# dkogan/libdogleg

Measured on AMD Instinct MI355X. Metric: trust-region steps/sec (fp64) at fixed (Nmeas,Nstate,nnz), higher is better.
Workload: dtype f64

## Files before the change

libdogleg_amd/capi.py:

```python
import ctypes as C
import os
import numpy as np

from .ctypes_defs import (Parameters2, CholmodSparse, Trace, TraceBuffer, BatchResult, BatchLoss, BatchBounds, BatchFit, JacobianReport, JacobianEntry,
                          CB_SPARSE, CB_DENSE, CB_PRODUCTS, dptr, iptr)

HERE = os.path.dirname(os.path.abspath(__file__))
LIB_PATH = os.environ.get("DLG_TEST_LIB") or os.path.join(HERE, "libdogleg_amd.so")

DLG_OK = 0
DLG_DENSE, DLG_SPARSE, DLG_DENSE_PRODUCTS = 0, 1, 2
FLAG_PACKED, FLAG_UPPER = 1, 2
KIND_CAUCHY, KIND_GN, KIND_INTERP = 0, 1, 2
VEC_P, VEC_X, VEC_JTX, VEC_CAUCHY, VEC_GN, VEC_STEP, VEC_J, VEC_X_OWN, VEC_J_OWN = range(9)

ALLREDUCE_FN = C.CFUNCTYPE(C.c_int, C.c_void_p, C.c_size_t, C.c_void_p)

BACKEND_SYMBOLS = [
    "dlg_last_error", "dlg_device_count", "dlg_backend_create", "dlg_backend_destroy",
    "dlg_backend_set_stream", "dlg_backend_get_stream", "dlg_backend_set_shard",
    "dlg_sparse_set_pattern", "dlg_sparse_stats", "dlg_sparse_schedule", "dlg_sparse_leaf_rows_stats", "dlg_point_set_p", "dlg_point_upload",
    "dlg_point_upload_products", "dlg_point_bind_device", "dlg_point_eval", "dlg_cauchy",
    "dlg_factorize", "dlg_solve_gn", "dlg_gauss_newton", "dlg_cauchy_gauss_newton", "dlg_make_step",
    "dlg_expected_improvement", "dlg_step", "dlg_take_step", "dlg_solve_with_factor",
# ... 832 lines not shown

    def init_rccl(self, rank, nranks, unique_id):
        buf = C.create_string_buffer(unique_id, 128)
        _ck(self.L.dlg_backend_init_rccl(self.h, rank, nranks, C.cast(buf, C.c_void_p)), "init_rccl")

    def set_noop_comm(self, on=True):
        _ck(self.L.dlg_backend_set_noop_comm(self.h, 1 if on else 0), "set_noop_comm")

    def comm_size(self):
        n = C.c_int()
        _ck(self.L.dlg_backend_comm_size(self.h, C.byref(n)), "comm_size")
        return n.value

    def set_pattern(self, Jp, Ji):
        Jp = np.ascontiguousarray(Jp, dtype=np.int32)
        Ji = np.ascontiguousarray(Ji, dtype=np.int32)
        _ck(self.L.dlg_sparse_set_pattern(self.h, iptr(Jp), iptr(Ji)), "set_pattern")

    def stats(self):
        a, b = C.c_long(), C.c_long()
        c, d = C.c_int(), C.c_int()
        e = C.c_double()
        _ck(self.L.dlg_sparse_stats(self.h, C.byref(a), C.byref(b), C.byref(c), C.byref(d), C.byref(e)),
            "stats")
        return dict(nnz_JtJ_lower=a.value, nnz_L=b.value, n_supernodes=c.value, n_levels=d.value,
                    factor_flops=e.value)

    def schedule(self):
        a, b, c = C.c_int(), C.c_int(), C.c_int()
        _ck(self.L.dlg_sparse_schedule(self.h, C.byref(a), C.byref(b), C.byref(c)), "schedule")
        return dict(n_levels=a.value, persist_level0=b.value, persist_items=c.value)

    def leaf_rows_stats(self):
        v = (C.c_long * 4)()
        _ck(self.L.dlg_sparse_leaf_rows_stats(self.h, v, 4), "leaf_rows_stats")
        return dict(lean_launches=v[0], materialized=v[1], raw=bool(v[2]), lean_levels=v[3])

    def set_p(self, slot, p):
        p = np.ascontiguousarray(p, dtype=np.float64)
        _ck(self.L.dlg_point_set_p(self.h, slot, dptr(p)), "set_p")

    def upload(self, slot, x, J):
        x = np.ascontiguousarray(x, dtype=np.float64)
        J = np.ascontiguousarray(J, dtype=np.float64)
        self._keep = [x, J]
        _ck(self.L.dlg_point_upload(self.h, slot, dptr(x), dptr(J)), "upload")

    def upload_products(self, slot, norm2x, Jtx, JtJ):
        Jtx = np.ascontiguousarray(Jtx, dtype=np.float64)
        JtJ = np.ascontiguousarray(JtJ, dtype=np.float64)
        self._keep = [Jtx, JtJ]
        _ck(self.L.dlg_point_upload_products(self.h, slot, norm2x, dptr(Jtx), dptr(JtJ)), "upload")

    def bind_device(self, slot, x_ptr, J_ptr):
        _ck(self.L.dlg_point_bind_device(self.h, slot, C.c_void_p(x_ptr), C.c_void_p(J_ptr)), "bind")

    def eval(self, slot):
        a, b = C.c_double(), C.c_double()
        _ck(self.L.dlg_point_eval(self.h, slot, C.byref(a), C.byref(b)), "eval")
        return a.value, b.value

    def cauchy(self, slot):
        a = C.c_double()
        _ck(self.L.dlg_cauchy(self.h, slot, C.byref(a)), "cauchy")
        return a.value

    def factorize(self, slot, lam=0.0):
        ok = C.c_int()
        _ck(self.L.dlg_factorize(self.h, slot, lam, C.byref(ok)), "factorize")
# ... 199 lines not shown
```

libdogleg_amd/csrc/backend.hip:

```cpp
#include "dlg_internal.h"

static thread_local char g_err[1024] = "";
#include <chrono>
#include <atomic>
#include <mutex>
namespace {
constexpr int DLG_TURN_DEV = 64;
std::mutex g_turn_mu;
std::atomic<int> g_turn_live[DLG_TURN_DEV];
hipEvent_t g_turn_ev[DLG_TURN_DEV];
dlg_backend* g_turn_owner[DLG_TURN_DEV];
}
DlgRegionTurn::DlgRegionTurn(dlg_backend* b_) : b(b_), on(false)
{
  const int d = b->device & (DLG_TURN_DEV - 1);
  if(g_turn_live[d].load(std::memory_order_relaxed) <= 1 || !b->ev_region) return;
  on = true;
  g_turn_mu.lock();
  if(g_turn_owner[d] && g_turn_owner[d] != b && g_turn_ev[d]) (void)hipEventSynchronize(g_turn_ev[d]);
}
DlgRegionTurn::~DlgRegionTurn()
{
  if(!on) return;
  const int d = b->device & (DLG_TURN_DEV - 1);
// ... 175 lines not shown

  auto fail = [&](int rc) { dlg_backend_destroy(b); return rc; };
#define TRY_HIP(call) do { hipError_t e_ = (call); if(e_ != hipSuccess) { \
    dlg_set_error("%s:%d: %s -> %s", __FILE__, __LINE__, #call, hipGetErrorString(e_)); \
    return fail(DLG_ERR_HIP); } } while(0)

  TRY_HIP(hipStreamCreateWithFlags(&b->stream, hipStreamNonBlocking));
  b->own_stream = true;
  TRY_HIP(hipStreamCreateWithFlags(&b->copy_stream, hipStreamNonBlocking));
  TRY_HIP(hipEventCreateWithFlags(&b->ev_step, hipEventDisableTiming));
  TRY_HIP(hipEventCreateWithFlags(&b->ev_copy, hipEventDisableTiming));
  TRY_HIP(hipStreamCreateWithFlags(&b->aux_stream, hipStreamNonBlocking));
  TRY_HIP(hipEventCreateWithFlags(&b->ev_fork, hipEventDisableTiming));
  TRY_HIP(hipEventCreateWithFlags(&b->ev_join, hipEventDisableTiming));
  TRY_HIP(hipEventCreateWithFlags(&b->ev_region, hipEventDisableTiming));
  turn_register(b); b->turn_registered = true;
  TRY_HIP(hipMalloc(&b->d_join, sizeof(int)*2));
  TRY_HIP(hipMemsetAsync(b->d_join, 0, sizeof(int)*2, b->stream));
  b->overlap = getenv("DOGLEG_AMD_NO_OVERLAP") == nullptr;
  b->fuse_eval = getenv("DOGLEG_AMD_NO_FUSED_EVAL") == nullptr;
  TRY_HIP(hipMalloc(&b->d_scal, sizeof(double)*dlg_backend::NSCAL));
  TRY_HIP(hipMemsetAsync(b->d_scal, 0, sizeof(double)*dlg_backend::NSCAL, b->stream));
  TRY_HIP(hipHostMalloc(&b->h_scal, sizeof(double)*dlg_backend::NSCAL));
  TRY_HIP(hipHostMalloc(&b->h_part, sizeof(double)*dlg_backend::HPART_CAP));
  b->host_finals = getenv("DOGLEG_AMD_DEVICE_FINALS") == nullptr;
  {
    dlg_backend::Knobs& k = b->knobs;
    k.potrf_steps = getenv("DOGLEG_AMD_POTRF_STEPS") != nullptr;
    k.trsv_steps = getenv("DOGLEG_AMD_TRSV_STEPS") != nullptr;
    k.no_abandon = getenv("DOGLEG_AMD_NO_ABANDON") != nullptr;
    k.ei_jpass = getenv("DOGLEG_AMD_EI_JPASS") != nullptr;
    k.no_between = getenv("DOGLEG_AMD_NO_BETWEEN") != nullptr;
    k.no_k8_predict = getenv("DOGLEG_AMD_NO_K8_PREDICT") != nullptr;
    if(const char* e = getenv("DOGLEG_AMD_DEBUG_EI_FLIP")) b->ei_flip = atoi(e);
    if(getenv("DOGLEG_AMD_DEBUG_HANDOFF_TIMEOUT")) { b->handoff_skew = 1; b->handoff_spins = 256; }
    (void)hipDeviceGetAttribute(&b->ncu, hipDeviceAttributeMultiprocessorCount, device);
    if(b->ncu <= 0) b->ncu = 256;
  }
  TRY_HIP(hipHostMalloc(&b->h_vec, sizeof(double)*(size_t)Nstate));
  TRY_HIP(hipMalloc(&b->d_work, sizeof(double)*(size_t)Nstate));
  const size_t N = (size_t)Nstate, M = (size_t)Nmeas;
  for(int s = 0; s < 2; s++)
  {
    DlgSlot& S = b->slot[s];
    TRY_HIP(hipMalloc(&S.p,      sizeof(double)*N));
    TRY_HIP(hipMalloc(&S.Jt_x,   sizeof(double)*(N + 8)));
    TRY_HIP(hipMalloc(&S.cauchy, sizeof(double)*N));
    TRY_HIP(hipMalloc(&S.gn,     sizeof(double)*(N + 8)));
    TRY_HIP(hipMalloc(&S.step,   sizeof(double)*N));
    TRY_HIP(hipMemsetAsync(S.p, 0, sizeof(double)*N, b->stream));
    TRY_HIP(hipMemsetAsync(S.step, 0, sizeof(double)*N, b->stream));
    if(solve_type != DLG_DENSE_PRODUCTS && M > 0) TRY_HIP(hipMalloc(&S.x, sizeof(double)*M));
    TRY_HIP(hipMalloc(&S.J, sizeof(double)*dlg_j_doubles(b)));
  }
#undef TRY_HIP
  int rc = (solve_type == DLG_SPARSE) ? sparse_create(b) : dense_create(b);
  if(rc != DLG_OK) return fail(rc);
  if(hipStreamSynchronize(b->stream) != hipSuccess)
  { dlg_set_error("stream sync failed during create"); return fail(DLG_ERR_HIP); }
  *out = b;
  return DLG_OK;
}

extern "C" void dlg_backend_destroy(dlg_backend_t* b)
{
  if(!b) return;
// ... 372 lines not shown
```

libdogleg_amd/csrc/dlg_internal.h:

```cpp
#pragma once
#include <hip/hip_runtime.h>
#include <hip/hip_ext.h>
#include <cstdio>
#include <cstdlib>
#include <cstring>
#include <cstdarg>
#include <cmath>
#include <vector>
#include <string>
#include "../../include/dlg_backend.h"

void dlg_set_error(const char* fmt, ...);

#define DLG_HIP(call)                                                              \
  do {                                                                             \
    hipError_t e__ = (call);                                                       \
    if(e__ != hipSuccess) {                                                        \
      dlg_set_error("%s:%d: %s -> %s", __FILE__, __LINE__, #call,                  \
                    hipGetErrorString(e__));                                       \
      return DLG_ERR_HIP;                                                          \
    }                                                                              \
  } while(0)

#define DLG_CHECK(call)                                                            \
// ... 43 lines not shown
  bool presolve = false;
  bool pre_rejected = false;
  bool factor_ahead = false;
  bool pre_split = false;
  bool prof_cont = false;
  int  pre_slot = -1, pre_held = -1; double pre_lambda = 0.0, pre_hint = 0.0; bool pre_hint_valid = false, pre_hint_input = false;
  DlgSlot slot[2];

  double* d_scal = nullptr;
  double* h_scal = nullptr;
  int* fork_gate = nullptr; int fork_gate_epoch = 0;
  bool defer_tail = false, tail_pending = false;
  int tail_nb = 0;
  double tail_inner = 0.0, tail_value = 0.0;
  double* h_tail = nullptr; int h_tail_cap = 0;
  unsigned long sync_mark = 0, tail_mark = 0;
  bool factor_doomed = false;
  static constexpr int IDENT_SLOT = 3, GB_SLOT = 13;
  static constexpr double IDENT_RATIO_MAX = 212.0;
  static constexpr double IDENT_ERR_MAX = 1e-12;
  bool ident_predict = false;
  bool ei_from_system = false; double pivot_ratio = NAN;
  int ei_flip = 0, ei_count = 0;
  bool tail_ident = false, tail_no_fold = false; double tail_nJs = 0.0;
  bool p_side_pending = false;
  dlg_between_fn between_fn = nullptr; void* between_cookie = nullptr; bool between_armed = false, between_ran = false, between_redone = false;
  int early_slot = -1; const double* early_x = nullptr; const double* early_J = nullptr;
  static constexpr int NSCAL = 16;
  int handoff_spins = 0, handoff_skew = 0;
  struct Knobs
  {
    bool potrf_steps = false, trsv_steps = false, no_abandon = false, ei_jpass = false, no_between = false, no_k8_predict = false;
    int touch_wg = 512;
  } knobs;
  int ncu = 256;

  double* d_part = nullptr;
  size_t  part_cap = 0;
  double* d_gnpart = nullptr;
  struct PendingFinal { size_t off; int nb, nsum, nmax, dst, stride; };
  static constexpr size_t HPART_CAP = 16384;
  double* h_part = nullptr;
  size_t  h_part_used = 0;
  std::vector<PendingFinal> pending;
  bool    host_finals = true;

  double* h_vec = nullptr;

  double* G = nullptr;
  double* Linv = nullptr;
  int* potrf_flag = nullptr; int potrf_epoch = 0; int* trsv_flag = nullptr; double* trsv_y = nullptr; double* trsv_x = nullptr; int trsv_epoch = 0;
  double* slabs = nullptr;
  size_t  slabs_bytes = 0;
  int*    d_info = nullptr;
  int*    h_info = nullptr;
  bool    defer_factor_sync = false;
  double* d_work = nullptr;
  DevScratch solve_scr, lev_scr;
  struct CovPlan* cov = nullptr; int cov_last = -1;
  struct SelInv* selinv = nullptr;

  SparseSym* sym = nullptr;

  int row0 = 0, row1 = 0;
  int mloc = 0;
  int part_rank = 0, part_nranks = 1;
// ... 287 lines not shown
```

libdogleg_amd/csrc/sparse_factor.hip:

```cpp
#include "sparse_internal.h"
#include "panel_factor.h"
#include "factor_tail.h"

namespace {
#ifdef DLG_FL_PROFILE
constexpr int FL_PROF_WG = 4096;
__device__ long long g_fl_prof[32*FL_PROF_WG*8];
__device__ long long g_fl_add[FL_PROF_WG*4];
#define FL_ADD_STAMP(k) do { if(HANDOFF && threadIdx.x == 0 && blockIdx.x < FL_PROF_WG) g_fl_add[blockIdx.x*4 + (k)] = wall_clock64(); } while(0)
#define FL_STAMP(k) do { if(threadIdx.x == 0 && blockIdx.x < FL_PROF_WG) g_fl_prof[((prof_lvl & 31)*FL_PROF_WG + blockIdx.x)*8 + (k)] = wall_clock64(); } while(0)
#else
#define FL_STAMP(k)
#define FL_ADD_STAMP(k)
#endif

template <int NT, bool UT_LDS, bool HANDOFF = false>
__device__ __forceinline__ void mf_add_children(double* P, double* Wt, int ntri, int nch, int ch0,
                                                MfChild rc, const MfChild* __restrict__ mf_rec,
                                                const double* uscr, const uint16_t* __restrict__ mf_dst, int tid,
                                                int* pr_flag = nullptr, int pr_epoch = 0, DlgHandoff ho = DlgHandoff{nullptr, 0, 0}, int z0 = 0)
{
  constexpr int MF_SLOTS = (NT >= 512) ? 20 : 16;
  const int lane = tid & 63;
  for(int e = z0 + tid; e < ntri; e += NT) Wt[e] = 0.0;
// ... 1196 lines not shown
                         Y->upart, (const int*)Y->d_info);
    if(H.part_nranks > 1 && l == H.cut_level) { DLG_LAUNCH_CHECK(); DLG_CHECK(sparse_partition_reduce(b)); }
  }
  if(!H.ms_sn.empty())
    hipLaunchKernelGGL(k_copy_top, dim3((unsigned)H.ms_sn.size()), dim3(TPB), 0, st, Y->ms_sn, Y->sn_c0,
                       Y->sn_rowptr, Y->sn_lx, Y->sn_top, Y->Lx, Y->top_scr, (const int*)Y->d_info);
  DLG_LAUNCH_CHECK();
  return DLG_OK;
}

int sparse_leaf_rows_materialize(dlg_backend* b)
{
  SparseSym* Y = b->sym;
  if(!Y || !Y->Lx || !Y->leaf_rows.raw(Y->Lx)) return DLG_OK;
  const SymHost& H = Y->H;
  const int slot = Y->leaf_rows.slot(Y->Lx);
  for(int l = 0; l < H.nlevels; l++)
  {
    const int n = H.fw_lvl_ptr[l+1] - H.fw_lvl_ptr[l];
    if(!Y->leaf_lean[l] || n == 0) continue;
    hipLaunchKernelGGL(HIP_KERNEL_NAME(k_leaf_rows_materialize<256>), dim3(n), dim3(256), Y->fac.lds[l], b->stream,
                       Y->fw_item + H.fw_lvl_ptr[l], Y->Lx, Y->leaf_rd + (size_t)slot*H.N, (const int*)Y->d_info);
  }
  DLG_LAUNCH_CHECK();
  Y->leaf_rows.materialize(Y->Lx);
  return DLG_OK;
}
extern "C" int dlg_sparse_leaf_rows_stats(dlg_backend_t* b, long* stats, int nstats)
{
  if(!b || !b->sym || !stats) { dlg_set_error("no symbolic analysis yet"); return DLG_ERR_STATE; }
  const SparseSym* Y = b->sym;
  long lean = 0;
  for(char c : Y->leaf_lean) lean += c;
  const long v[] = { Y->leaf_rows.lean_launches, Y->leaf_rows.materialized, Y->leaf_rows.raw(Y->Lx) ? 1L : 0L, lean };
  for(int i = 0; i < nstats && i < 4; i++) stats[i] = v[i];
  return DLG_OK;
}

extern "C" int dlg_sparse_region_probe(int N, int M, const int* colptr, const int* rowidx, int ncu, long* stats, int nstats)
{
  SymHost H;
  char err[512];
  if(sym_analyze(H, N, M, colptr, rowidx, 0, M, err, sizeof(err))) { dlg_set_error("symbolic analysis: %s", err); return DLG_ERR_ARG; }
  const RegionKnobs K = region_knobs_env(ncu);
  FacLevels L;
  if(fac_level_params(H, L, err, sizeof(err))) { dlg_set_error("%s", err); return DLG_ERR_ARG; }
  const RegionPlan R = region_plan(H, L, 1, H.nlevels - 1, K);
  long checked[2];
  if(region_check(H, R, checked, err, sizeof(err))) { dlg_set_error("%s", err); return DLG_ERR_STATE; }
  const long v[] = { (long)R.level0, (long)(H.fw_lvl_ptr[H.nlevels] - H.fw_lvl_ptr[std::min(R.level0, H.nlevels)]),
                     (long)R.nwg, (long)R.lds, checked[0], checked[1], (long)region_plan_hash(R), (long)fac_levels_hash(L) };
  for(int i = 0; i < nstats && i < 8; i++) stats[i] = v[i];
  return DLG_OK;
}
```

libdogleg_amd/csrc/sparse_internal.h:

```cpp
#pragma once
#include "dlg_internal.h"
#include "sparse_symbolic.h"
#include "sparse_region.h"
#include "leaf_rows_state.h"

namespace {
constexpr int JFL_SEG = 16;
constexpr int NV_CHUNK = 2048;

constexpr int TPB = 256;
constexpr int LDS_BUDGET = SYM_LDS_BUDGET;
constexpr int FAC_LDS_BUDGET = SYM_FAC_LDS_BUDGET;

__device__ __forceinline__ double wave_sum(double v)
{
#pragma unroll
  for(int o = 32; o > 0; o >>= 1) v += __shfl_down(v, o, 64);
  return v;
}

template <int NT, int U, class LoadF, class StoreF>
__device__ __forceinline__ void batched_copy(int total, int tid, LoadF ld, StoreF st)
{
  for(int base = 0; base < total; base += U*NT)
// ... 45 lines not shown
  int *jtx_fin_ptr = nullptr, *jtx_fin_blk = nullptr;
  int *jtx_fin_short = nullptr, *jtx_fin_long = nullptr; int n_fin_short = 0, n_fin_long = 0;
  AsmRho* asm_rho = nullptr; AsmPair* asm_pair = nullptr; AsmSlot* asm_slot = nullptr;
  AsmBatch* asm_batch = nullptr; AsmTask* asm_ctask = nullptr; AsmFin* asm_cfin = nullptr;
  bool asm_pent_ok = false;
  uint32_t* asm_pent = nullptr;
  AsmShape* asm_shape = nullptr; AsmKG* asm_kg = nullptr; AsmMTask* asm_mtask = nullptr; int* asm_tdest = nullptr;
  int *jf_ptr = nullptr, *jf_ent = nullptr, *jf_var0 = nullptr, *jf_w = nullptr, *jf_short = nullptr, *jf_long = nullptr;
  double* jf_lpart = nullptr; int* jf_lcnt = nullptr;
  const double* fin_pending_rhs = nullptr; const double* spec_aug_rhs = nullptr; bool info_clean = false;
  double* fin_pending_Lx = nullptr;
  bool spare_dirty = false, spare_zeroed = false; hipStream_t spare_stream = nullptr;
  double* jtp = nullptr;
  AsmFin2* asm_fin2 = nullptr; int64_t* asm_fin2_list = nullptr; AsmRun* asm_run = nullptr; int* asm_pdest = nullptr;
  int *rl_ptr = nullptr, *rl_pos = nullptr, *perm = nullptr, *col_sn = nullptr;
  int *fw_sn = nullptr, *fw_r0 = nullptr, *fw_r1 = nullptr, *ms_sn = nullptr; int64_t* sn_top = nullptr;
  int *sn_bd_ptr = nullptr, *sn_bd_col = nullptr;
  double* top_scr = nullptr;
  const double* aug_rhs = nullptr;
  int *Jp = nullptr, *Ji = nullptr;
  int *gat_rows = nullptr, *gat_src = nullptr;
  int *nv_chunk = nullptr; int n_nv_chunks = 0;
  double *Lx = nullptr, *scr = nullptr, *ywork = nullptr, *asm_part = nullptr, *jtx_part = nullptr;
  int *d_info = nullptr, *h_info = nullptr;
  bool info_armed = false;
  bool zero_fail_seen = false; int64_t* leaf_diag = nullptr; int* leaf_diag_col = nullptr; int n_leaf_diag = 0;
  double* intact_Lx = nullptr; const double* intact_J = nullptr; int intact_slot = -1; double intact_lambda = 0.0;
  const double* fac_J = nullptr; int fac_slot = -1;
  bool fac_pending = false;
  size_t nnz_loc = 0;
  uint32_t* ar_idx = nullptr; double* ar_buf = nullptr; size_t ar_n = 0;
  FacLevels fac;
  std::vector<int> slv_lds, bwd_lds, bwd_nt, bwd_bd, bwd_pmx;
  int64_t* red_off = nullptr; int* red_len = nullptr; int* red_kind = nullptr; int64_t* red_dst = nullptr;
  int n_red_seg = 0; size_t red_n = 0; double* red_buf = nullptr;
  double* colmask = nullptr; int* sn_owner = nullptr;
  int64_t* augpos = nullptr;
  int *xl_sn = nullptr;
  double* held_Lx = nullptr; const double* held_aug = nullptr; double held_lambda = 0.0;
  LeafRowsState leaf_rows; std::vector<char> leaf_lean; double* leaf_rd = nullptr;
  double cur_lambda = 0.0;
  double *ms_scr = nullptr, *ms_y = nullptr; int ms_lds_f = 0, ms_lds_b = 0;
  typedef ReachPlan LevPlan;
  LevPlan lev[2];
  int* lev_iperm = nullptr; std::vector<int> lev_jp, lev_ji; int lev_lds = 0;
  double* Lx_spec = nullptr; hipEvent_t ev_spec = nullptr, ev_spec_fork = nullptr;
  bool spec_inflight = false, spec_valid = false; int spec_slot = -1; const double* spec_J = nullptr;
  int64_t touch_off = 0, touch_n = 0;
  int bw_level0 = 1 << 30, bw_lds = 0, bw_n = 0;
  SolveItem* slv_item_pr = nullptr; int* bwd_flag = nullptr; int bwd_epoch = 0; double* bwd_xh = nullptr;
  PrRegion top, lo; double* pr_acc = nullptr;
  int64_t* clr_off = nullptr; int64_t* clr_len = nullptr; int n_clr = 0; bool clr_partial_ok = false; double* lz_ok[2] = {nullptr, nullptr};
  int64_t* aug_of_var = nullptr; char* jf_listed = nullptr;
  int aug_fused_epoch = 0; const double* spec_aug_fused = nullptr;
  int* fin_flag = nullptr; int fin_epoch = 0, fin_side_owed = 0; bool fin_side_sched_ok = false; hipStream_t fin_main = nullptr;
  int bwd_xb_cap = 12288;
  double* diag_mm = nullptr; int n_diag_mm = 0;
  std::vector<void*> allocs;
};

int sparse_assemble(dlg_backend* b, int s, double lambda);
int sparse_partition_reduce(dlg_backend* b);
int sparse_assemble_speculative(dlg_backend* b, int s);
int sparse_eval_assemble(dlg_backend* b, int s, int* done);
int sparse_assemble_finish(dlg_backend* b);
int sparse_zero_spare(dlg_backend* b, hipStream_t ordered_for);
// ... 5 lines not shown
```

libdogleg_amd/csrc/sparse_solve.hip:

```cpp
#include "sparse_internal.h"

namespace {
#ifdef DLG_FL_PROFILE
__device__ long long g_bw_prof[64*8];
__device__ long long g_bw_chain[256*8];
#define BW_STAMP(k) do { if(threadIdx.x == 0 && blockIdx.x == 0) g_bw_prof[(prof_lvl & 63)*8 + (k)] = clock64(); \
                         if(threadIdx.x == 0 && pr_flag && blockIdx.x < 256) g_bw_chain[blockIdx.x*8 + (k)] = wall_clock64(); } while(0)
#else
#define BW_STAMP(k)
#endif

__global__ void __launch_bounds__(TPB) k_solve_fwd_level(const int* __restrict__ lvl_sn,
                                                         const int* __restrict__ sn_c0,
                                                         const int* __restrict__ sn_rowptr,
                                                         const int64_t* __restrict__ sn_lx,
                                                         const int* __restrict__ sn_scr,
                                                         const int* __restrict__ rl_ptr,
                                                         const int* __restrict__ rl_pos,
                                                         const int* __restrict__ perm,
                                                         const double* __restrict__ Lx,
                                                         const double* __restrict__ rhs,
                                                         double* __restrict__ scr,
                                                         double* __restrict__ ywork)
{
// ... 31 lines not shown
      __syncthreads();
      if(lane == 0) red[wv] = sum;
      __syncthreads();
      if(tid == 0) y[j] = rhs[perm[k]] - ((red[0] + red[1]) + (red[2] + red[3]));
    }
    else if((j & 3) == wv)
    {
      double sum = 0.0;
      for(int e = e0 + lane; e < e1; e += 64) sum += scr[rl_pos[e]];
      sum = wave_sum(sum);
      if(lane == 0) y[j] = rhs[perm[k]] - sum;
    }
  }
  __syncthreads();
  double yi = (tid < w) ? y[tid] : 0.0;
  for(int j = 0; j < w; j++)
  {
    if(tid == j) y[j] = yi / lds[j + j*ldp];
    __syncthreads();
    if(tid > j && tid < w) yi -= lds[tid + j*ldp]*y[j];
  }
  __syncthreads();
  for(int j = tid; j < w; j += TPB) ywork[c0 + j] = y[j];
  const int r = nrows - w - 1;
  double* u = scr + sn_scr[s];
  for(int i = tid; i < r; i += TPB)
  {
    double sum = 0.0;
#pragma unroll 8
    for(int j = 0; j < w; j++) sum += L[w + i + (size_t)j*nrows]*y[j];
    u[i] = sum;
  }
}
template <int BWD_NT, bool BD_ONLY>
__global__ void __launch_bounds__(BWD_NT, BD_ONLY ? 4 : 1) k_solve_bwd_level(const SolveItem* __restrict__ items,
                                                            const int* __restrict__ sn_rows,
                                                            const int* __restrict__ perm,
                                                            const double* __restrict__ Lx,
                                                            double* __restrict__ ywork,
                                                            double* __restrict__ out, int use_aug,
                                                            const int* __restrict__ sn_bd_col, int top_lds, int xb_cap,
                                                            int* pr_flag, int pr_epoch, const int* __restrict__ info, DlgHandoff ho,
                                                            double* xh, int xh_n, double* __restrict__ mm, int rows_raw)
{
  extern __shared__ __attribute__((aligned(16))) double lds[];
  __shared__ int s_skip;
  double dmin = 1e300, dmax = 0.0;
  if(threadIdx.x == 0) s_skip = *info != 0x7fffffff;
  constexpr int NW = BWD_NT/64;
  typedef const __attribute__((address_space(1))) double* gcd_t;
  typedef __attribute__((address_space(1))) double* gd_t;
  auto ldx = [&](const double* p) -> double { return pr_flag ? __hip_atomic_load((gcd_t)p, __ATOMIC_RELAXED, __HIP_MEMORY_SCOPE_AGENT) : *p; };
  constexpr unsigned long long X_EMPTY = 0x7FF8DEADBEEF0002ull;
  typedef __attribute__((address_space(1))) unsigned long long* gu_t;
  const bool xh_on = pr_flag != nullptr && xh != nullptr && ho.skew == 0;
  unsigned long long* xcur = reinterpret_cast<unsigned long long*>(xh) + (size_t)(pr_epoch & 1)*xh_n;
  auto put_xh = [&](int col, double v) {
    if(xh_on) __hip_atomic_store((gu_t)(xcur + col), (unsigned long long)__double_as_longlong(v), __ATOMIC_RELAXED, __HIP_MEMORY_SCOPE_AGENT); };
  auto take_xh = [&](int col) -> double {
    unsigned long long u; int spins = 0;
    while((u = __hip_atomic_load((gu_t)(xcur + col), __ATOMIC_RELAXED, __HIP_MEMORY_SCOPE_AGENT)) == X_EMPTY)
    { __builtin_amdgcn_s_sleep(1); if(++spins > ho.spins) { atomicOr(ho.status, DLG_HANDOFF_SOLVE); u = 0; break; } }
    return __longlong_as_double((long long)u); };

  const int prof_lvl = top_lds >> 8; (void)prof_lvl;
  top_lds &= 1;
  BW_STAMP(0);
  const SolveItem it = items[blockIdx.x];
  const int c0 = it.c0, w = it.w, nrows = it.nrows;
  if(xh_on && (int)threadIdx.x < w) reinterpret_cast<unsigned long long*>(xh)[(size_t)(1 - (pr_epoch & 1))*xh_n + c0 + threadIdx.x] = X_EMPTY;
  const int* rows = sn_rows + it.rowoff;
  const double* L = Lx + it.lx;
  const int tid = threadIdx.x, lane = tid & 63, wv = tid >> 6;
  const int r = nrows - w - 1;
  const int nblk = (w + 7) >> 3;
  const bool xb_lds = r <= xb_cap;
  double* xb = lds;
  double* xs = lds + (xb_lds ? ((r + 1) & ~1) : 0);
  double* T = xs + 256;
  double* rhs = T + nblk*64;
  double* xp = rhs + 16;
  double* Lt = xp + 8*256;
  const int ldt = w | 1;
  const int MW = (w + 15) & ~15;
  double* Mx = Lt + (top_lds ? w*ldt : 0);
  const int nmem = BD_ONLY ? max(it.nbd, 1) : it.nbd;
  const int myrow = (tid < r) ? rows[w + tid] : 0;
  double myrhs = 0.0; int myperm = 0;
  if(tid < w) { myrhs = use_aug ? L[(nrows - 1) + (size_t)tid*nrows] : ywork[c0 + tid]; myperm = perm[c0 + tid]; }
  constexpr bool LEAN = BWD_NT == 256;
  constexpr int MV_SLOTS = LEAN ? 20 : 24;
  const int mv_cols = min(BWD_NT, max(w, 64)), mv_parts = BWD_NT/mv_cols;
  const int mv_j = tid % mv_cols, mv_p = tid/mv_cols;
  const int mv_len = (r + mv_parts - 1)/mv_parts;
  const int mv_i0 = mv_p*mv_len, mv_i1 = min(r, mv_i0 + mv_len);
  const bool mv_thread = mv_len <= MV_SLOTS && xb_lds;
  const bool mv_on = mv_thread && mv_j < w && mv_p < mv_parts;
  const double* mv_L = L + (size_t)min(mv_j, w - 1)*nrows + w;
  double mv[MV_SLOTS];
  {
    typedef double bw_v2d __attribute__((ext_vector_type(2)));
    typedef bw_v2d bw_v2d_u __attribute__((aligned(8)));
#pragma unroll
    for(int q = 0; q < MV_SLOTS; q += 2)
    {
      if(mv_on && mv_i0 + q + 1 < mv_i1) { const bw_v2d t = *reinterpret_cast<const bw_v2d_u*>(mv_L + mv_i0 + q); mv[q] = t.x; mv[q + 1] = t.y; }
      else { mv[q] = (mv_on && mv_i0 + q < mv_i1) ? mv_L[mv_i0 + q] : 0.0; mv[q + 1] = 0.0; }
    }
  }
  if(!BD_ONLY)
  for(int e = tid; e < (nmem > 0 ? 0 : nblk*64); e += BWD_NT)
  {
    const int j0 = (e >> 6)*8, a = (e >> 3) & 7, b = e & 7;
    const bool valid = a >= b && j0 + a < w;
    double v = valid ? L[(j0 + a) + (size_t)(j0 + b)*nrows] : 0.0;
    if(a == b && valid) { dmin = fmin(dmin, v); dmax = fmax(dmax, v); }
    if(a == b) v = valid ? 1.0/v : 1.0;
    T[e] = v;
  }
  if(!BD_ONLY && top_lds && nmem == 0)
  {
    const int cp_rows = min(BWD_NT, (w + 63) & ~63), cp_ng = BWD_NT/cp_rows, cp_g = tid/cp_rows;
    for(int i = tid - cp_g*cp_rows; i < w && cp_g < cp_ng; i += cp_rows)
      for(int j0 = cp_g; j0 <= i; j0 += 16*cp_ng)
      {
        double v[16];
#pragma unroll
        for(int u = 0; u < 16; u++) v[u] = (j0 + u*cp_ng <= i) ? L[i + (size_t)(j0 + u*cp_ng)*nrows] : 0.0;
#pragma unroll
        for(int u = 0; u < 16; u++) if(j0 + u*cp_ng <= i) Lt[i + (j0 + u*cp_ng)*ldt] = v[u];
      }
  }
  double Lm[8][8];
  int m0 = 0, nbm = 0;
  if(nmem > 0 && tid < nmem)
  {
    if(it.rsv > 0) { m0 = tid*it.rsv; nbm = it.rsv; }
    else
    {
      const int* mcol = sn_bd_col + it.bd0;
      m0 = mcol[tid]; nbm = ((tid + 1 < nmem) ? mcol[tid + 1] : w) - m0;
    }
  }
  if(nmem > 0)
  {
#pragma unroll
    for(int a = 0; a < 8; a++)
#pragma unroll
      for(int b = 0; b <= a; b++) Lm[a][b] = (a < nbm) ? L[(m0 + a) + (size_t)(m0 + b)*nrows] : (a == b ? 1.0 : 0.0);
    if(mm)
    {
#pragma unroll
      for(int a = 0; a < 8; a++) if(a < nbm) { dmin = fmin(dmin, Lm[a][a]); dmax = fmax(dmax, Lm[a][a]); }
    }
  }
  if(mm && (nmem > 0 ? 64*wv < nmem : wv < nblk))
  {
#pragma unroll
    for(int o = 32; o > 0; o >>= 1) { dmin = fmin(dmin, __shfl_down(dmin, o, 64)); dmax = fmax(dmax, __shfl_down(dmax, o, 64)); }
    if(lane == 0) { mm[(8*blockIdx.x + wv)*2] = dmin; mm[(8*blockIdx.x + wv)*2 + 1] = dmax; }
  }
  BW_STAMP(1);
  const bool premul = it.rsv != 0 && !BD_ONLY && nmem == 0 && pr_flag != nullptr && it.pflag >= 0;
  if(premul)
  {
    __syncthreads();
    double ti[8];
    const bool ton = tid < 8*nblk;
    if(ton)
    {
      const double* Tb = T + (tid >> 3)*64;
      const int c = tid & 7;
      double Lb[8][8];
#pragma unroll
      for(int a = 0; a < 8; a++)
#pragma unroll
        for(int b2 = 0; b2 <= a; b2++) Lb[a][b2] = Tb[a*8 + b2];
#pragma unroll
      for(int i = 0; i < 8; i++)
      {
        double v = 0.0;
#pragma unroll
        for(int k = 0; k < i; k++) v -= (k >= c) ? Lb[i][k]*ti[k] : 0.0;
        ti[i] = (i == c) ? Lb[i][i] : ((i > c) ? v*Lb[i][i] : 0.0);
      }
    }
    __syncthreads();
    if(ton)
    {
// ... 52 lines not shown
  else if(xb_lds)
  {
    if(tid < r) xb[tid] = ldx(ywork + myrow);
    for(int i = tid + BWD_NT; i < r; i += BWD_NT) xb[i] = ldx(ywork + rows[w + i]);
  }
  __syncthreads();
  if(s_skip)
  {
    if(tid < w) put_xh(c0 + tid, 0.0);
    if(pr_flag && tid == 0) __hip_atomic_store(pr_flag + blockIdx.x, pr_epoch, __ATOMIC_RELAXED, __HIP_MEMORY_SCOPE_AGENT);
    return;
  }
  BW_STAMP(2);
  double tinv[8];
  const bool tinv_on = !BD_ONLY && nmem == 0 && tid < 8*nblk && !premul;
  if(tinv_on)
  {
    const double* Tb = T + (tid >> 3)*64;
    const int c = tid & 7;
    double Lb[8][8];
#pragma unroll
    for(int a = 0; a < 8; a++)
#pragma unroll
      for(int b = 0; b <= a; b++) Lb[a][b] = Tb[a*8 + b];
#pragma unroll
    for(int i = 0; i < 8; i++)
    {
      double v = 0.0;
#pragma unroll
      for(int k = 0; k < i; k++) v -= (k >= c) ? Lb[i][k]*tinv[k] : 0.0;
      tinv[i] = (i == c) ? Lb[i][i] : ((i > c) ? v*Lb[i][i] : 0.0);
    }
  }
  if(mv_thread)
  {
    double acc = 0.0;
#pragma unroll
    for(int q = 0; q < MV_SLOTS; q++) acc += mv[q]*((mv_i0 + q < mv_i1) ? xb[mv_i0 + q] : 0.0);
    if(mv_on) xp[mv_p*256 + mv_j] = acc;
  }
  else
  {
    for(int e = 256 + tid; e < mv_parts*256; e += BWD_NT) xp[e] = 0.0;
    for(int jg = 4*wv; jg < w; jg += 4*NW)
    {
      const double* Lj = L + (size_t)jg*nrows + w;
      const int nc = min(4, w - jg);
      double acc[4] = {0.0, 0.0, 0.0, 0.0};
#pragma unroll 2
      for(int i = lane; i < r; i += 64)
      {
        const double x = xb_lds ? xb[i] : ldx(ywork + rows[w + i]);
#pragma unroll
        for(int c = 0; c < 4; c++) acc[c] += ((c < nc) ? Lj[i + (size_t)c*nrows] : 0.0)*x;
      }
#pragma unroll
      for(int c = 0; c < 4; c++)
      {
        const double sum = wave_sum(acc[c]);
        if(lane == 0 && c < nc) xp[jg + c] = sum;
      }
    }
  }
  double Lz[4][4];
  if(LEAN && rows_raw)
  {
#pragma unroll
    for(int a = 0; a < 4; a++)
#pragma unroll
      for(int b = 0; b <= a; b++) Lz[a][b] = (tid < nmem && a < nbm) ? L[(m0 + a) + (size_t)(m0 + b)*nrows] : (a == b ? 1.0 : 0.0);
  }
  __syncthreads();
  BW_STAMP(3);
  if(tinv_on)
  {
    double* Tb = T + (tid >> 3)*64;
    const int c = tid & 7;
#pragma unroll
    for(int i = 0; i < 8; i++) if(i >= c) Tb[i*8 + c] = tinv[i];
  }
  if(nmem > 0)
  {
    if(tid < w)
    {
      double sum = 0.0;
      for(int p = 0; p < mv_parts; p++) sum += xp[p*256 + tid];
      if(rows_raw) { xs[tid] = sum; xp[tid] = myrhs; }
      else xs[tid] = myrhs - sum;
    }
    __syncthreads();
    if(rows_raw && tid < nmem)
    {
      double z[4];
#pragma unroll
      for(int a = 0; a < 4; a++)
      {
        double v = (a < nbm) ? xs[m0 + a] : 0.0;
#pragma unroll
        for(int b = 0; b < a; b++) v -= (LEAN ? Lz[a][b] : Lm[a][b])*z[b];
        z[a] = v/(LEAN ? Lz[a][a] : Lm[a][a]);
      }
#pragma unroll
      for(int a = 0; a < 4; a++) if(a < nbm) xs[m0 + a] = xp[m0 + a] - z[a];
    }
    if(LEAN)
    {
      if(tid < nmem)
        for(int a = nbm - 1; a >= 0; a--)
        {
          const double* Lc = L + (size_t)(m0 + a)*nrows + m0;
          double v = xs[m0 + a];
          for(int b = a + 1; b < nbm; b++) v -= Lc[b]*xs[m0 + b];
          xs[m0 + a] = v/Lc[a];
        }
    }
    else if(tid < nmem)
    {
      double xk[8];
#pragma unroll
      for(int a = 7; a >= 0; a--)
      {
        double v = (a < nbm) ? xs[m0 + a] : 0.0;
#pragma unroll
        for(int b = a + 1; b < 8; b++) v -= Lm[b][a]*xk[b];
        xk[a] = v/Lm[a][a];
      }
#pragma unroll
      for(int a = 0; a < 8; a++) if(a < nbm) xs[m0 + a] = xk[a];
    }
    __syncthreads();
    if(tid < w)
    {
      put_xh(c0 + tid, xs[tid]);
      if(pr_flag) __hip_atomic_store((gd_t)(ywork + c0 + tid), xs[tid], __ATOMIC_RELAXED, __HIP_MEMORY_SCOPE_AGENT);
      else ywork[c0 + tid] = xs[tid];
      out[myperm] = xs[tid];
    }
    if(pr_flag)
// ... 172 lines not shown
  }
  hipMemcpyFromSymbol(h, HIP_SYMBOL(g_bw_prof), sizeof(h));
  for(int l = 0; l < nlevels && l < 64; l++)
    fprintf(stderr, "bwd level %2d: issue %6lld  gather+barrier %6lld  matvec %6lld  solve %6lld  store %6lld cycles | to first barrier %6lld, in it %6lld, rest of the loop %6lld\n", l,
            h[l*8+1] - h[l*8], h[l*8+2] - h[l*8+1], h[l*8+3] - h[l*8+2], h[l*8+4] - h[l*8+3], h[l*8+5] - h[l*8+4],
            h[l*8+6] - h[l*8+3], h[l*8+7] - h[l*8+6], h[l*8+4] - h[l*8+7]);
}
#endif
int sparse_touch_factor(dlg_backend* b, hipStream_t st)
{
  SparseSym* Y = b->sym;
  if(!Y || !Y->touch_n) return DLG_OK;
  const int nwg = b->knobs.touch_wg;
  hipLaunchKernelGGL(k_touch, dim3(nwg), dim3(TPB), 0, st, reinterpret_cast<const double2*>(Y->Lx + Y->touch_off),
                     (size_t)Y->touch_n/2, Y->ywork);
  DLG_LAUNCH_CHECK();
  return DLG_OK;
}
static SolveItem solve_item(const SymHost& H, int s)
{
  SolveItem it;
  it.c0 = H.sn_c0[s]; it.w = H.sn_c0[s+1] - H.sn_c0[s]; it.nrows = H.sn_rowptr[s+1] - H.sn_rowptr[s];
  it.rowoff = H.sn_rowptr[s]; it.lx = H.sn_lx[s]; it.bd0 = H.sn_bd_ptr[s]; it.nbd = H.sn_bd_ptr[s+1] - H.sn_bd_ptr[s];
  it.pflag = -1; it.rsv = 0;
  return it;
}

int sparse_solve_setup(dlg_backend* b)
{
  SparseSym* Y = b->sym;
  const SymHost& H = Y->H;
  const long xb_cap = env_int("DOGLEG_AMD_BWD_XB_CAP", 12288);
  Y->bwd_xb_cap = (int)xb_cap;
  Y->slv_lds.assign(H.nlevels, 0); Y->bwd_lds.assign(H.nlevels, 0); Y->bwd_nt.assign(H.nlevels, 512); Y->bwd_bd.assign(H.nlevels, 0); Y->bwd_pmx.assign(H.nlevels, 0);
  for(int l = 0; l < H.nlevels; l++)
  {
    long maxw = 0, mb = 0;
    for(int i = H.lvl_ptr[l]; i < H.lvl_ptr[l+1]; i++)
    {
      const int s = H.lvl_sn[i];
      const long wv = H.sn_c0[s+1] - H.sn_c0[s], nr = H.sn_rowptr[s+1] - H.sn_rowptr[s];
      if(wv > maxw) maxw = wv;
      const long rb = nr - wv - 1;
      const long need = (rb <= xb_cap ? rb + 3 : 0) + 256 + ((wv + 7)/8)*64 + 16 + 8*256;
      if(need > mb) mb = need;
    }
    if(maxw > 256) { dlg_set_error("supernode of width %ld is too wide for the backward-solve kernel", maxw); return DLG_ERR_ARG; }
    Y->slv_lds[l] = (int)(maxw*(maxw | 1)*8);
    if(Y->slv_lds[l] > LDS_BUDGET) { dlg_set_error("supernode of width %ld is too wide for the solve kernels", maxw); return DLG_ERR_ARG; }
    if(mb*8 > LDS_BUDGET) { dlg_set_error("supernode too large for the backward-solve kernel (%ld doubles)", mb); return DLG_ERR_ARG; }
    Y->bwd_lds[l] = (int)(mb*8);
    Y->bwd_pmx[l] = 0;
    {
      long pm = 0;
      for(int i = H.lvl_ptr[l]; i < H.lvl_ptr[l+1]; i++)
      {
        const int s = H.lvl_sn[i];
        const long wv = H.sn_c0[s+1] - H.sn_c0[s];
        if(H.sn_bd_ptr[s+1] == H.sn_bd_ptr[s]) pm = std::max(pm, ((wv + 7)/8)*8*((wv + 15) & ~15L));
      }
      if(pm > 0 && !getenv("DOGLEG_AMD_NO_PREMUL") && (long)Y->bwd_lds[l] + pm*8 <= LDS_BUDGET) Y->bwd_pmx[l] = (int)(pm*8);
    }
    Y->bwd_nt[l] = (maxw <= 128 && H.lvl_ptr[l+1] - H.lvl_ptr[l] >= 512) ? 256 : 512;
    bool allbd = true;
    for(int i = H.lvl_ptr[l]; i < H.lvl_ptr[l+1]; i++) { const int s = H.lvl_sn[i]; if(H.sn_bd_ptr[s+1] == H.sn_bd_ptr[s]) allbd = false; }
    Y->bwd_bd[l] = allbd ? 1 : 0;
    if(Y->bwd_nt[l] != 512 || Y->bwd_bd[l]) Y->bwd_pmx[l] = 0;
    Y->bwd_lds[l] += Y->bwd_pmx[l];
  }
  {
    std::vector<SolveItem> items(H.xl_sn.size());
    for(int k = 0; k < (int)H.xl_sn.size(); k++)
    {
      const int s = H.xl_sn[k];
      SolveItem& it = items[k];
      it = solve_item(H, s);
      it.rsv = Y->bwd_pmx[H.sn_level[s]] ? 1 : 0;
      if(it.nbd > 0)
      {
        const int* mc = &H.sn_bd_col[it.bd0];
        const int wd0 = (it.nbd > 1 ? mc[1] : it.w) - mc[0];
        bool same = mc[0] == 0;
        for(int m = 0; m < it.nbd && same; m++) if(((m + 1 < it.nbd) ? mc[m+1] : it.w) - mc[m] != wd0 || mc[m] != m*wd0) same = false;
        it.rsv = same ? wd0 : 0;
      }
    }
    DLG_CHECK(upload(Y->slv_item, items)); Y->allocs.push_back(Y->slv_item);
    std::vector<double> none(16*std::max<size_t>(items.size(), 1));
    for(size_t i = 0; i < none.size(); i += 2) { none[i] = 1e300; none[i + 1] = 0.0; }
    DLG_CHECK(upload(Y->diag_mm, none)); Y->allocs.push_back(Y->diag_mm);
    Y->n_diag_mm = 8*(int)items.size();
  }
  {
    int64_t lo = -1, hi = 0;
    for(int i = H.lvl_ptr[0]; i < H.lvl_ptr[1]; i++)
    {
      const int s = H.lvl_sn[i];
      const int64_t a = H.sn_lx[s], e = a + (int64_t)(H.sn_rowptr[s+1] - H.sn_rowptr[s])*(H.sn_c0[s+1] - H.sn_c0[s]);
      if(lo < 0 || a < lo) lo = a;
// ... 21 lines not shown
    {
      std::vector<SolveItem> items;
      std::vector<int> pos(H.nsn, -1);
      for(int l = H.nlevels - 1; l >= l0; l--)
        for(int k = H.xl_ptr[l]; k < H.xl_ptr[l+1]; k++)
        {
          const int s = H.xl_sn[k];
          SolveItem it = solve_item(H, s);
          it.rsv = Y->bwd_pmx[l] ? 1 : 0;
          if(it.nbd > 0) it.rsv = 0;
          if(it.nrows - it.w - 1 > 0)
          {
            const int prow = H.sn_rows[H.sn_rowptr[s] + it.w];
            const int ps = H.col_sn[prow];
            it.pflag = pos[ps];
            if(it.pflag < 0) { dlg_set_error("internal error: the parent of supernode %d is not part of the persistent backward launch", s); return DLG_ERR_ARG; }
          }
          pos[s] = (int)items.size();
          items.push_back(it);
        }
      Y->bw_level0 = l0; Y->bw_n = (int)items.size(); Y->bw_lds = std::max(ldsb, 84*1024);
      DLG_CHECK(upload(Y->slv_item_pr, items)); Y->allocs.push_back(Y->slv_item_pr);
      std::vector<unsigned long long> empty(2*(size_t)H.N, 0x7FF8DEADBEEF0002ull);
      DLG_HIP(hipMalloc(&Y->bwd_xh, sizeof(double)*empty.size())); Y->allocs.push_back(Y->bwd_xh);
      DLG_HIP(hipMemcpy(Y->bwd_xh, empty.data(), sizeof(double)*empty.size(), hipMemcpyHostToDevice));
      DLG_HIP(hipMalloc(&Y->bwd_flag, sizeof(int)*items.size())); Y->allocs.push_back(Y->bwd_flag);
      DLG_HIP(hipMemsetAsync(Y->bwd_flag, 0, sizeof(int)*items.size(), b->stream));
      Y->bwd_epoch = 0;
    }
  }
  for(int l = 0; l < H.nlevels; l++)
    if(Y->leaf_lean[l] && (l >= Y->bw_level0 || !Y->bwd_bd[l])) Y->leaf_lean[l] = 0;
  for(const void* k : { (const void*)&k_solve_fwd_level, (const void*)&k_solve_bwd_level<256, false>,
                        (const void*)&k_solve_bwd_level<256, true>, (const void*)&k_solve_bwd_level<512, false> })
    DLG_HIP(hipFuncSetAttribute(k, hipFuncAttributeMaxDynamicSharedMemorySize, LDS_BUDGET));
  return DLG_OK;
}

static double* bwd_diag_mm(const dlg_backend* b, int l)
{
  const SparseSym* Y = b->sym;
  return (Y->diag_mm && !b->knobs.ei_jpass) ? Y->diag_mm + 16*(size_t)Y->H.xl_ptr[l] : (double*)nullptr;
}
static void launch_bwd_level(dlg_backend* b, int nt, bool bd, int grid, int lds, const SolveItem* items, double* out, int use_aug,
                             int l, int* flag, int epoch, double* xh, int nxh)
{
  SparseSym* Y = b->sym;
  double* mm = bwd_diag_mm(b, l);
  const int rows_raw = (Y->leaf_lean[l] && Y->leaf_rows.raw(Y->Lx)) ? 1 : 0;
#define DLG_BW_LAUNCH(...) hipLaunchKernelGGL(HIP_KERNEL_NAME(k_solve_bwd_level<__VA_ARGS__>), dim3(grid), dim3(nt), lds, b->stream, \
                                              items, Y->sn_rows, Y->perm, Y->Lx, Y->ywork, out, use_aug, Y->sn_bd_col, 256*l, Y->bwd_xb_cap, \
                                              flag, epoch, Y->d_info, dlg_handoff(b, 1 << 21), xh, nxh, mm, rows_raw)
  if(nt == 256 && bd) DLG_BW_LAUNCH(256, true);
  else if(nt == 256) DLG_BW_LAUNCH(256, false);
  else { nt = 512; DLG_BW_LAUNCH(512, false); }
#undef DLG_BW_LAUNCH
}

int sparse_solve(dlg_backend* b, const double* rhs, double* out)
{
  SparseSym* Y = b->sym;
  if(!Y) { dlg_set_error("dlg_sparse_set_pattern must be called first"); return DLG_ERR_STATE; }
  const SymHost& H = Y->H;
  hipStream_t st = b->stream;
  const int use_aug = (Y->aug_rhs != nullptr && Y->aug_rhs == rhs) ? 1 : 0;
  if(H.part_nranks > 1 && !use_aug)
  { dlg_set_error("with a subtree partition only the right-hand side that rode along with the factorisation (Jt x) can be solved for"); return DLG_ERR_STATE; }
  if(!use_aug) DLG_CHECK(sparse_leaf_rows_materialize(b));
  for(int l = 0; l < H.nlevels && !use_aug; l++)
  {
    const int n = H.xl_ptr[l+1] - H.xl_ptr[l];
    if(n > 0)
      hipLaunchKernelGGL(k_solve_fwd_level, dim3(n), dim3(TPB), Y->slv_lds[l], st, Y->xl_sn + H.xl_ptr[l],
                         Y->sn_c0, Y->sn_rowptr, Y->sn_lx, Y->sn_scr, Y->rl_ptr, Y->rl_pos, Y->perm,
                         Y->Lx, rhs, Y->scr, Y->ywork);
  }
  if(H.part_nranks > 1) DLG_HIP(hipMemsetAsync(out, 0, sizeof(double)*(size_t)H.N, st));
  int ltop = H.nlevels - 1;
  if(Y->bw_level0 < H.nlevels)
  {
    DlgRegionTurn turn(b);
    launch_bwd_level(b, 512, false, Y->bw_n, Y->bw_lds, Y->slv_item_pr, out, use_aug, Y->bw_level0, Y->bwd_flag, ++Y->bwd_epoch, Y->bwd_xh, H.N);
    ltop = Y->bw_level0 - 1;
  }
  for(int l = ltop; l >= 0; l--)
  {
    const int n = H.xl_ptr[l+1] - H.xl_ptr[l];
    if(n > 0) launch_bwd_level(b, Y->bwd_nt[l], Y->bwd_bd[l], n, Y->bwd_lds[l], Y->slv_item + H.xl_ptr[l], out, use_aug, l, (int*)nullptr, 0, (double*)nullptr, 0);
  }
  DLG_LAUNCH_CHECK();
  if(H.part_nranks > 1)
  {
    const bool room = out == b->slot[0].gn || out == b->slot[1].gn;
    const double* extra = room ? b->fold_scalar : nullptr;
    hipLaunchKernelGGL(k_mask_vec, dim3(dlg_cdiv(H.N, TPB)), dim3(TPB), 0, st, out, Y->colmask, H.N, extra);
    DLG_LAUNCH_CHECK();
    DLG_CHECK(dlg_allreduce_dev(b, out, (size_t)H.N + (extra ? 1 : 0)));
    if(extra) { b->fold_result = out + H.N; b->fold_scalar = nullptr; }
  }
  return DLG_OK;
}
```

Measured before the change: 1905.

## Add lean raw-rows backward-solve kernel variant for narrow leaf levels

Adds a third instantiation of the backward level solve for leaf levels whose diagonal blocks are at most 4 wide and whose row data is raw. The variant drops the T/rhs LDS regions and the 8x8 block path, and solves each 4x4 diagonal block directly in registers. It also trims the per-block LDS request and raises the launch-bounds occupancy hint to 6, so more workgroups can be resident per CU. It is on by default through a knob, and adds stats counters. The cost is more template code, plus a risk of register spills under the tighter occupancy bound.

Measured after the change: 1883. -1.2%, worse.

```diff
diff --git a/libdogleg_amd/capi.py b/libdogleg_amd/capi.py
--- a/libdogleg_amd/capi.py
+++ b/libdogleg_amd/capi.py
@@ -888,9 +888,10 @@
         return dict(n_levels=a.value, persist_level0=b.value, persist_items=c.value)
 
     def leaf_rows_stats(self):
-        v = (C.c_long * 4)()
-        _ck(self.L.dlg_sparse_leaf_rows_stats(self.h, v, 4), "leaf_rows_stats")
-        return dict(lean_launches=v[0], materialized=v[1], raw=bool(v[2]), lean_levels=v[3])
+        v = (C.c_long * 6)()
+        _ck(self.L.dlg_sparse_leaf_rows_stats(self.h, v, 6), "leaf_rows_stats")
+        return dict(lean_launches=v[0], materialized=v[1], raw=bool(v[2]), lean_levels=v[3],
+                    bwd_raw4_launches=v[4], bwd_raw4_levels=v[5])
 
     def set_p(self, slot, p):
         p = np.ascontiguousarray(p, dtype=np.float64)
diff --git a/libdogleg_amd/csrc/backend.hip b/libdogleg_amd/csrc/backend.hip
--- a/libdogleg_amd/csrc/backend.hip
+++ b/libdogleg_amd/csrc/backend.hip
@@ -231,6 +231,7 @@
     k.ei_jpass = getenv("DOGLEG_AMD_EI_JPASS") != nullptr;
     k.no_between = getenv("DOGLEG_AMD_NO_BETWEEN") != nullptr;
     k.no_k8_predict = getenv("DOGLEG_AMD_NO_K8_PREDICT") != nullptr;
+    if(const char* e = getenv("DOGLEG_AMD_BWD_RAW4")) k.bwd_raw4 = atoi(e) != 0;
     if(const char* e = getenv("DOGLEG_AMD_DEBUG_EI_FLIP")) b->ei_flip = atoi(e);
     if(getenv("DOGLEG_AMD_DEBUG_HANDOFF_TIMEOUT")) { b->handoff_skew = 1; b->handoff_spins = 256; }
     (void)hipDeviceGetAttribute(&b->ncu, hipDeviceAttributeMultiprocessorCount, device);
diff --git a/libdogleg_amd/csrc/dlg_internal.h b/libdogleg_amd/csrc/dlg_internal.h
--- a/libdogleg_amd/csrc/dlg_internal.h
+++ b/libdogleg_amd/csrc/dlg_internal.h
@@ -99,6 +99,7 @@
   {
     bool potrf_steps = false, trsv_steps = false, no_abandon = false, ei_jpass = false, no_between = false, no_k8_predict = false;
     int touch_wg = 512;
+    bool bwd_raw4 = true;
   } knobs;
   int ncu = 256;
 
diff --git a/libdogleg_amd/csrc/sparse_factor.hip b/libdogleg_amd/csrc/sparse_factor.hip
--- a/libdogleg_amd/csrc/sparse_factor.hip
+++ b/libdogleg_amd/csrc/sparse_factor.hip
@@ -1252,8 +1252,10 @@
   const SparseSym* Y = b->sym;
   long lean = 0;
   for(char c : Y->leaf_lean) lean += c;
-  const long v[] = { Y->leaf_rows.lean_launches, Y->leaf_rows.materialized, Y->leaf_rows.raw(Y->Lx) ? 1L : 0L, lean };
-  for(int i = 0; i < nstats && i < 4; i++) stats[i] = v[i];
+  long fit4 = 0;
+  for(int c : Y->bwd_bd) fit4 += c == 2;
+  const long v[] = { Y->leaf_rows.lean_launches, Y->leaf_rows.materialized, Y->leaf_rows.raw(Y->Lx) ? 1L : 0L, lean, Y->bwd_raw4_launches, fit4 };
+  for(int i = 0; i < nstats && i < 6; i++) stats[i] = v[i];
   return DLG_OK;
 }
 
diff --git a/libdogleg_amd/csrc/sparse_internal.h b/libdogleg_amd/csrc/sparse_internal.h
--- a/libdogleg_amd/csrc/sparse_internal.h
+++ b/libdogleg_amd/csrc/sparse_internal.h
@@ -101,6 +101,7 @@
   uint32_t* ar_idx = nullptr; double* ar_buf = nullptr; size_t ar_n = 0;
   FacLevels fac;
   std::vector<int> slv_lds, bwd_lds, bwd_nt, bwd_bd, bwd_pmx;
+  std::vector<int> bwd_lds4; long bwd_raw4_launches = 0;
   int64_t* red_off = nullptr; int* red_len = nullptr; int* red_kind = nullptr; int64_t* red_dst = nullptr;
   int n_red_seg = 0; size_t red_n = 0; double* red_buf = nullptr;
   double* colmask = nullptr; int* sn_owner = nullptr;
diff --git a/libdogleg_amd/csrc/sparse_solve.hip b/libdogleg_amd/csrc/sparse_solve.hip
--- a/libdogleg_amd/csrc/sparse_solve.hip
+++ b/libdogleg_amd/csrc/sparse_solve.hip
@@ -87,8 +87,8 @@
     u[i] = sum;
   }
 }
-template <int BWD_NT, bool BD_ONLY>
-__global__ void __launch_bounds__(BWD_NT, BD_ONLY ? 4 : 1) k_solve_bwd_level(const SolveItem* __restrict__ items,
+template <int BWD_NT, bool BD_ONLY, bool RAW4 = false>
+__global__ void __launch_bounds__(BWD_NT, RAW4 ? 6 : (BD_ONLY ? 4 : 1)) k_solve_bwd_level(const SolveItem* __restrict__ items,
                                                             const int* __restrict__ sn_rows,
                                                             const int* __restrict__ perm,
                                                             const double* __restrict__ Lx,
@@ -98,6 +98,8 @@
                                                             int* pr_flag, int pr_epoch, const int* __restrict__ info, DlgHandoff ho,
                                                             double* xh, int xh_n, double* __restrict__ mm, int rows_raw)
 {
+  static_assert(!RAW4 || (BD_ONLY && BWD_NT == 256), "RAW4 is the lean leaf level's instantiation");
+  if(RAW4) { rows_raw = 1; pr_flag = nullptr; xh = nullptr; }
   extern __shared__ __attribute__((aligned(16))) double lds[];
   __shared__ int s_skip;
   double dmin = 1e300, dmax = 0.0;
@@ -133,8 +135,8 @@
   double* xb = lds;
   double* xs = lds + (xb_lds ? ((r + 1) & ~1) : 0);
   double* T = xs + 256;
-  double* rhs = T + nblk*64;
-  double* xp = rhs + 16;
+  double* rhs = T + (RAW4 ? 0 : nblk*64);
+  double* xp = rhs + (RAW4 ? 0 : 16);
   double* Lt = xp + 8*256;
   const int ldt = w | 1;
   const int MW = (w + 15) & ~15;
@@ -197,7 +199,7 @@
       m0 = mcol[tid]; nbm = ((tid + 1 < nmem) ? mcol[tid + 1] : w) - m0;
     }
   }
-  if(nmem > 0)
+  if(nmem > 0 && !RAW4)
   {
 #pragma unroll
     for(int a = 0; a < 8; a++)
@@ -209,7 +211,7 @@
       for(int a = 0; a < 8; a++) if(a < nbm) { dmin = fmin(dmin, Lm[a][a]); dmax = fmax(dmax, Lm[a][a]); }
     }
   }
-  if(mm && (nmem > 0 ? 64*wv < nmem : wv < nblk))
+  if(!RAW4 && mm && (nmem > 0 ? 64*wv < nmem : wv < nblk))
   {
 #pragma unroll
     for(int o = 32; o > 0; o >>= 1) { dmin = fmin(dmin, __shfl_down(dmin, o, 64)); dmax = fmax(dmax, __shfl_down(dmax, o, 64)); }
@@ -328,11 +330,20 @@
       tinv[i] = (i == c) ? Lb[i][i] : ((i > c) ? v*Lb[i][i] : 0.0);
     }
   }
-  if(mv_thread)
+  if(mv_thread || RAW4)
   {
     double acc = 0.0;
-#pragma unroll
-    for(int q = 0; q < MV_SLOTS; q++) acc += mv[q]*((mv_i0 + q < mv_i1) ? xb[mv_i0 + q] : 0.0);
+    if(!RAW4 || mv_on)
+    {
+#pragma unroll
+      for(int q = 0; q < MV_SLOTS; q++)
+      {
+        const bool in = mv_i0 + q < mv_i1;
+        if(RAW4) { const double xv = xb[in ? mv_i0 + q : 0]; acc += mv[q]*(in ? xv : 0.0); }
+        else acc += mv[q]*(in ? xb[mv_i0 + q] : 0.0);
+        if(RAW4 && (q & 3) == 3) __builtin_amdgcn_sched_barrier(0);
+      }
+    }
     if(mv_on) xp[mv_p*256 + mv_j] = acc;
   }
   else
@@ -366,6 +377,14 @@
 #pragma unroll
       for(int b = 0; b <= a; b++) Lz[a][b] = (tid < nmem && a < nbm) ? L[(m0 + a) + (size_t)(m0 + b)*nrows] : (a == b ? 1.0 : 0.0);
   }
+  if(RAW4 && mm && 64*wv < nmem)
+  {
+#pragma unroll
+    for(int a = 0; a < 4; a++) if(tid < nmem && a < nbm) { dmin = fmin(dmin, Lz[a][a]); dmax = fmax(dmax, Lz[a][a]); }
+#pragma unroll
+    for(int o = 32; o > 0; o >>= 1) { dmin = fmin(dmin, __shfl_down(dmin, o, 64)); dmax = fmax(dmax, __shfl_down(dmax, o, 64)); }
+    if(lane == 0) { mm[(8*blockIdx.x + wv)*2] = dmin; mm[(8*blockIdx.x + wv)*2 + 1] = dmax; }
+  }
   __syncthreads();
   BW_STAMP(3);
   if(tinv_on)
@@ -385,7 +404,32 @@
       else xs[tid] = myrhs - sum;
     }
     __syncthreads();
-    if(rows_raw && tid < nmem)
+    if(RAW4)
+    {
+      if(tid < nmem)
+      {
+        double z[4], xk[4];
+#pragma unroll
+        for(int a = 0; a < 4; a++)
+        {
+          double v = (a < nbm) ? xs[m0 + a] : 0.0;
+#pragma unroll
+          for(int b = 0; b < a; b++) v -= Lz[a][b]*z[b];
+          z[a] = v/Lz[a][a];
+        }
+#pragma unroll
+        for(int a = 3; a >= 0; a--)
+        {
+          double v = (a < nbm) ? xp[m0 + a] - z[a] : 0.0;
+#pragma unroll
+          for(int b = a + 1; b < 4; b++) v -= Lz[b][a]*xk[b];
+          xk[a] = v/Lz[a][a];
+        }
+#pragma unroll
+        for(int a = 0; a < 4; a++) if(a < nbm) xs[m0 + a] = xk[a];
+      }
+    }
+    else if(rows_raw && tid < nmem)
     {
       double z[4];
 #pragma unroll
@@ -399,7 +443,8 @@
 #pragma unroll
       for(int a = 0; a < 4; a++) if(a < nbm) xs[m0 + a] = xp[m0 + a] - z[a];
     }
-    if(LEAN)
+    if(RAW4) { }
+    else if(LEAN)
     {
       if(tid < nmem)
         for(int a = nbm - 1; a >= 0; a--)
@@ -638,7 +683,7 @@
   const SymHost& H = Y->H;
   const long xb_cap = env_int("DOGLEG_AMD_BWD_XB_CAP", 12288);
   Y->bwd_xb_cap = (int)xb_cap;
-  Y->slv_lds.assign(H.nlevels, 0); Y->bwd_lds.assign(H.nlevels, 0); Y->bwd_nt.assign(H.nlevels, 512); Y->bwd_bd.assign(H.nlevels, 0); Y->bwd_pmx.assign(H.nlevels, 0);
+  Y->slv_lds.assign(H.nlevels, 0); Y->bwd_lds.assign(H.nlevels, 0); Y->bwd_nt.assign(H.nlevels, 512); Y->bwd_bd.assign(H.nlevels, 0); Y->bwd_pmx.assign(H.nlevels, 0); Y->bwd_lds4.assign(H.nlevels, 0);
   for(int l = 0; l < H.nlevels; l++)
   {
     long maxw = 0, mb = 0;
@@ -671,6 +716,22 @@
     bool allbd = true;
     for(int i = H.lvl_ptr[l]; i < H.lvl_ptr[l+1]; i++) { const int s = H.lvl_sn[i]; if(H.sn_bd_ptr[s+1] == H.sn_bd_ptr[s]) allbd = false; }
     Y->bwd_bd[l] = allbd ? 1 : 0;
+    if(allbd && Y->bwd_nt[l] == 256 && b->knobs.bwd_raw4)
+    {
+      bool narrow = true; long mb4 = 0;
+      for(int i = H.lvl_ptr[l]; i < H.lvl_ptr[l+1]; i++)
+      {
+        const int s = H.lvl_sn[i];
+        const long wv = H.sn_c0[s+1] - H.sn_c0[s], rb = H.sn_rowptr[s+1] - H.sn_rowptr[s] - wv - 1;
+        for(int m = H.sn_bd_ptr[s]; m < H.sn_bd_ptr[s+1]; m++)
+          if((m + 1 < H.sn_bd_ptr[s+1] ? H.sn_bd_col[m+1] : (int)wv) - H.sn_bd_col[m] > 4) narrow = false;
+        const long parts = 256/std::min(256L, std::max(wv, 64L));
+        if(rb > xb_cap || (rb + parts - 1)/parts > 20) narrow = false;
+        mb4 = std::max(mb4, rb + 3 + 256 + parts*256);
+      }
+      constexpr long LDS_SIXTH = ((160*1024/6) & ~255) - 64;
+      if(narrow) { Y->bwd_bd[l] = 2; Y->bwd_lds4[l] = (int)std::min((long)LDS_BUDGET, std::max(mb4*8, LDS_SIXTH)); }
+    }
     if(Y->bwd_nt[l] != 512 || Y->bwd_bd[l]) Y->bwd_pmx[l] = 0;
     Y->bwd_lds[l] += Y->bwd_pmx[l];
   }
@@ -758,7 +819,8 @@
   for(int l = 0; l < H.nlevels; l++)
     if(Y->leaf_lean[l] && (l >= Y->bw_level0 || !Y->bwd_bd[l])) Y->leaf_lean[l] = 0;
   for(const void* k : { (const void*)&k_solve_fwd_level, (const void*)&k_solve_bwd_level<256, false>,
-                        (const void*)&k_solve_bwd_level<256, true>, (const void*)&k_solve_bwd_level<512, false> })
+                        (const void*)&k_solve_bwd_level<256, true>, (const void*)&k_solve_bwd_level<256, true, true>,
+                        (const void*)&k_solve_bwd_level<512, false> })
     DLG_HIP(hipFuncSetAttribute(k, hipFuncAttributeMaxDynamicSharedMemorySize, LDS_BUDGET));
   return DLG_OK;
 }
@@ -768,7 +830,7 @@
   const SparseSym* Y = b->sym;
   return (Y->diag_mm && !b->knobs.ei_jpass) ? Y->diag_mm + 16*(size_t)Y->H.xl_ptr[l] : (double*)nullptr;
 }
-static void launch_bwd_level(dlg_backend* b, int nt, bool bd, int grid, int lds, const SolveItem* items, double* out, int use_aug,
+static void launch_bwd_level(dlg_backend* b, int nt, int bd, int grid, int lds, const SolveItem* items, double* out, int use_aug,
                              int l, int* flag, int epoch, double* xh, int nxh)
 {
   SparseSym* Y = b->sym;
@@ -777,7 +839,8 @@
 #define DLG_BW_LAUNCH(...) hipLaunchKernelGGL(HIP_KERNEL_NAME(k_solve_bwd_level<__VA_ARGS__>), dim3(grid), dim3(nt), lds, b->stream, \
                                               items, Y->sn_rows, Y->perm, Y->Lx, Y->ywork, out, use_aug, Y->sn_bd_col, 256*l, Y->bwd_xb_cap, \
                                               flag, epoch, Y->d_info, dlg_handoff(b, 1 << 21), xh, nxh, mm, rows_raw)
-  if(nt == 256 && bd) DLG_BW_LAUNCH(256, true);
+  if(nt == 256 && bd == 2 && rows_raw) { lds = Y->bwd_lds4[l]; Y->bwd_raw4_launches++; DLG_BW_LAUNCH(256, true, true); }
+  else if(nt == 256 && bd) DLG_BW_LAUNCH(256, true);
   else if(nt == 256) DLG_BW_LAUNCH(256, false);
   else { nt = 512; DLG_BW_LAUNCH(512, false); }
 #undef DLG_BW_LAUNCH
@@ -806,7 +869,7 @@
   if(Y->bw_level0 < H.nlevels)
   {
     DlgRegionTurn turn(b);
-    launch_bwd_level(b, 512, false, Y->bw_n, Y->bw_lds, Y->slv_item_pr, out, use_aug, Y->bw_level0, Y->bwd_flag, ++Y->bwd_epoch, Y->bwd_xh, H.N);
+    launch_bwd_level(b, 512, 0, Y->bw_n, Y->bw_lds, Y->slv_item_pr, out, use_aug, Y->bw_level0, Y->bwd_flag, ++Y->bwd_epoch, Y->bwd_xh, H.N);
     ltop = Y->bw_level0 - 1;
   }
   for(int l = ltop; l >= 0; l--)
```
